# stjude-rust-labs/ngs

Measured on NVIDIA B200. Metric: ngs qc records/sec, higher is better.
Workload: dtype u8/u64

## Files before the change

ngs_b200/csrc/inflate2.cuh:

```cuda
#pragma once
#include <cstdint>
#include <cuda_runtime.h>

#include "inflate_lane.cuh"

namespace ngsq {

constexpr int kDecBatch = 32;
constexpr int kDecWarps = 18;
constexpr int kDecThreads = kDecWarps * 32;
constexpr size_t kDecSmem = (size_t)kDecThreads * kSlabBytes;

__global__ void __launch_bounds__(kDecThreads, 1)
inflate_decode_kernel(uint8_t* __restrict__ out, const BlockDesc* __restrict__ blocks, uint32_t n_blocks,
                      uint32_t* __restrict__ queue, uint32_t* __restrict__ status, uint32_t* __restrict__ bitmap) {
  extern __shared__ __align__(16) uint8_t smem_raw[];
  const uint32_t lane = threadIdx.x & 31;
  Lane L;
  L.slab = smem_raw + (size_t)threadIdx.x * kSlabBytes;
  L.state = LS_IDLE;
  __shared__ uint32_t s_base_lut[64];
  if (threadIdx.x < 64) s_base_lut[threadIdx.x] = base_lut_entry(threadIdx.x);
  __syncthreads();
  L.lut = s_base_lut;
  const uint32_t static_blocks = gridDim.x * (uint32_t)kDecWarps * 32u;
  bool first = true;
  for (;;) {
    uint32_t base = 0;
    if (first) {
      base = ((threadIdx.x >> 5) * gridDim.x + blockIdx.x) * 32u;
      first = false;
    } else {
      if (lane == 0) base = static_blocks + atomicAdd(queue, 32u);
      base = __shfl_sync(0xFFFFFFFFu, base, 0);
    }
    if (base >= n_blocks) break;
    const uint32_t b = base + lane;
    if (b < n_blocks) L.begin_block(blocks[b], out, bitmap + (size_t)b * kBitmapWords);
    else L.state = LS_IDLE;
    while (__any_sync(0xFFFFFFFFu, L.state != LS_IDLE)) {
      if (L.state == LS_HEADER) L.header();
      __syncwarp();
#pragma unroll 1
      for (int it = 0; it < kDecBatch; ++it) {
        if (L.state == LS_DECODE) L.step();
        L.settle();
        if (!__any_sync(0xFFFFFFFFu, L.state == LS_DECODE)) break;
      }
      if (L.state == LS_DECODE && L.overran()) L.end_block(kBlkBadStream);
    }
    if (b < n_blocks && L.err) status[b] = L.err;
  }
}

constexpr int kResThreads = 256;
constexpr int kResWarps = kResThreads / 32;
constexpr int kResList = 352;

__device__ __forceinline__ uint2 load8_unaligned(const uint8_t* s, uint32_t n) {
  const uint32_t* a = reinterpret_cast<const uint32_t*>(reinterpret_cast<uintptr_t>(s) & ~uintptr_t(3));
  const uint32_t mis = (uint32_t)(reinterpret_cast<uintptr_t>(s) & 3);
  const uint32_t sh = mis * 8;
  const uint32_t w0 = a[0], w1 = a[1];
  uint32_t w2 = 0;
  if (mis + n > 8) w2 = a[2];
  return make_uint2(__funnelshift_r(w0, w1, sh), __funnelshift_r(w1, w2, sh));
}

__device__ __forceinline__ void store_bytes(uint8_t* d, uint2 v, uint32_t n) {
  d[0] = (uint8_t)v.x;
  if (n > 1) d[1] = (uint8_t)(v.x >> 8);
  if (n > 2) d[2] = (uint8_t)(v.x >> 16);
  if (n > 3) d[3] = (uint8_t)(v.x >> 24);
  if (n > 4) d[4] = (uint8_t)v.y;
  if (n > 5) d[5] = (uint8_t)(v.y >> 8);
  if (n > 6) d[6] = (uint8_t)(v.y >> 16);
  if (n > 7) d[7] = (uint8_t)(v.y >> 24);
}

__device__ __forceinline__ void resolve_copy(uint8_t* dst, uint32_t mlen, uint32_t dist) {
  uint32_t D = dist;
  for (uint32_t done = 0; done < mlen;) {
    const uint32_t n = min(min(8u, D), mlen - done);
    store_bytes(dst + done, load8_unaligned(dst + done - D, n), n);
    done += n;
    if (D < 8) D <<= 1;
  }
}

__global__ void __launch_bounds__(kResThreads)
inflate_resolve_kernel(uint8_t* __restrict__ out, const BlockDesc* __restrict__ blocks, uint32_t n_blocks,
                       const uint32_t* __restrict__ bitmap, const uint32_t* __restrict__ status) {
  __shared__ uint16_t s_pos[kResWarps][kResList];
  __shared__ uint2 s_rank[kResWarps][32];
  const uint32_t lane = threadIdx.x & 31, wic = threadIdx.x >> 5;
  const uint32_t n_warps = gridDim.x * kResWarps;
  uint16_t* list = s_pos[wic];
  for (uint32_t b = blockIdx.x * kResWarps + wic; b < n_blocks; b += n_warps) {
    if (status[b]) continue;
    const BlockDesc d = blocks[b];
    uint8_t* ob = out + d.out_off;
    const uint32_t* bmp = bitmap + (size_t)b * kBitmapWords;
    const uint32_t n_sw = (d.isize + 1023) >> 10;
    for (uint32_t sw = 0; sw < n_sw; ++sw) {
      uint32_t word = bmp[sw * 32 + lane];
      const uint32_t cnt = __popc(word);
      uint32_t incl = cnt;
#pragma unroll
      for (int o = 1; o < 32; o <<= 1) {
        uint32_t t = __shfl_up_sync(0xFFFFFFFFu, incl, o);
        if ((int)lane >= o) incl += t;
      }
      const uint32_t total = __shfl_sync(0xFFFFFFFFu, incl, 31);
      if (!total) continue;
      uint32_t o = incl - cnt;
      s_rank[wic][lane] = make_uint2(word, o);
      const uint32_t pbase = (sw << 10) + (lane << 5);
      while (word) {
        const uint32_t bit = __ffs(word) - 1;
        word &= word - 1;
        list[o++] = (uint16_t)(pbase + bit);
      }
      __syncwarp();
      uint32_t pos_n = 0xFFFFu, tok_n = 0;
      if (lane < total) {
        pos_n = list[lane];
        const uint8_t* t = ob + pos_n;
        tok_n = (uint32_t)t[0] | ((uint32_t)t[1] << 8) | ((uint32_t)t[2] << 16);
      }
      for (uint32_t base = 0; base < total; base += 32) {
        const bool active = base + lane < total;
        const uint32_t pos = pos_n, tok = tok_n;
        const uint32_t jn = base + 32 + lane;
        if (jn < total) {
          pos_n = list[jn];
          const uint8_t* t = ob + pos_n;
          tok_n = (uint32_t)t[0] | ((uint32_t)t[1] << 8) | ((uint32_t)t[2] << 16);
        }
        const uint32_t mlen = (tok & 255u) + 3u, dist = (tok >> 8) + 1u;
        const uint32_t dend = active ? pos + mlen : 0x20000u;
        const uint32_t s_lo = pos - dist, s_hi = s_lo + min(mlen, dist);
        const uint32_t W = sw << 10;
        const uint32_t x_lo = min(max(s_lo, W) - W, 1023u), x_hi = min(max(s_hi, W) - W, 1023u);
        const uint2 e_lo = s_rank[wic][x_lo >> 5], e_hi = s_rank[wic][x_hi >> 5];
        const uint32_t r_lo = e_lo.y + __popc(e_lo.x & ((1u << (x_lo & 31)) - 1u));
        const uint32_t r_hi = e_hi.y + __popc(e_hi.x & ((1u << (x_hi & 31)) - 1u));
        const int pl = (int)r_lo - 1 - (int)base;
        const uint32_t prev_end = __shfl_sync(0xFFFFFFFFu, dend, pl & 31);
        const int lo = max((int)r_lo - (int)base - ((pl >= 0 && prev_end > s_lo) ? 1 : 0), 0), hi = (int)r_hi - (int)base;
        uint32_t dep = 0;
        if (active && hi > lo) dep = ((1u << hi) - 1u) & ~((1u << lo) - 1u) & ((1u << lane) - 1u);
        uint32_t done = __ballot_sync(0xFFFFFFFFu, !active);
        while (done != 0xFFFFFFFFu) {
          const bool ready = !((done >> lane) & 1u) && (dep & ~done) == 0;
          if (ready) resolve_copy(ob + pos, mlen, dist);
          __syncwarp();
          done |= __ballot_sync(0xFFFFFFFFu, ready);
        }
      }
      __syncwarp();
    }
  }
}

}
```

Measured before the change: 377.9 million.

## Interleave match copies chunk-wise across lanes and map one warp per block

The resolve kernel no longer runs a per-lane `resolve_copy` loop inside the warp's ready/ballot loop. Each ready lane now copies one chunk of at most 8 bytes per warp iteration, and a match is marked done only when its remaining length reaches zero. This removes the divergence where a whole warp waited on one long copy. The grid-stride loop is dropped in favour of one warp per BGZF block, launch bounds ask for 8 resident blocks per SM, and token loads and byte stores use word/mask forms. The one-warp-per-block mapping is correct only if the host launches enough blocks to cover every BGZF block; that launch code is not shown here.

```diff
diff --git a/ngs_b200/csrc/inflate2.cuh b/ngs_b200/csrc/inflate2.cuh
--- a/ngs_b200/csrc/inflate2.cuh
+++ b/ngs_b200/csrc/inflate2.cuh
@@ -68,98 +68,93 @@
 }
 
 __device__ __forceinline__ void store_bytes(uint8_t* d, uint2 v, uint32_t n) {
-  d[0] = (uint8_t)v.x;
-  if (n > 1) d[1] = (uint8_t)(v.x >> 8);
-  if (n > 2) d[2] = (uint8_t)(v.x >> 16);
-  if (n > 3) d[3] = (uint8_t)(v.x >> 24);
-  if (n > 4) d[4] = (uint8_t)v.y;
-  if (n > 5) d[5] = (uint8_t)(v.y >> 8);
-  if (n > 6) d[6] = (uint8_t)(v.y >> 16);
-  if (n > 7) d[7] = (uint8_t)(v.y >> 24);
+  const uint32_t m = (1u << n) - 1u;
+  if (m & 1u) d[0] = (uint8_t)v.x;
+  if (m & 2u) d[1] = (uint8_t)(v.x >> 8);
+  if (m & 4u) d[2] = (uint8_t)(v.x >> 16);
+  if (m & 8u) d[3] = (uint8_t)(v.x >> 24);
+  if (m & 16u) d[4] = (uint8_t)v.y;
+  if (m & 32u) d[5] = (uint8_t)(v.y >> 8);
+  if (m & 64u) d[6] = (uint8_t)(v.y >> 16);
+  if (m & 128u) d[7] = (uint8_t)(v.y >> 24);
 }
 
-__device__ __forceinline__ void resolve_copy(uint8_t* dst, uint32_t mlen, uint32_t dist) {
-  uint32_t D = dist;
-  for (uint32_t done = 0; done < mlen;) {
-    const uint32_t n = min(min(8u, D), mlen - done);
-    store_bytes(dst + done, load8_unaligned(dst + done - D, n), n);
-    done += n;
-    if (D < 8) D <<= 1;
-  }
-}
-
-__global__ void __launch_bounds__(kResThreads)
+__global__ void __launch_bounds__(kResThreads, 8)
 inflate_resolve_kernel(uint8_t* __restrict__ out, const BlockDesc* __restrict__ blocks, uint32_t n_blocks,
                        const uint32_t* __restrict__ bitmap, const uint32_t* __restrict__ status) {
   __shared__ uint16_t s_pos[kResWarps][kResList];
   __shared__ uint2 s_rank[kResWarps][32];
   const uint32_t lane = threadIdx.x & 31, wic = threadIdx.x >> 5;
-  const uint32_t n_warps = gridDim.x * kResWarps;
   uint16_t* list = s_pos[wic];
-  for (uint32_t b = blockIdx.x * kResWarps + wic; b < n_blocks; b += n_warps) {
-    if (status[b]) continue;
-    const BlockDesc d = blocks[b];
-    uint8_t* ob = out + d.out_off;
-    const uint32_t* bmp = bitmap + (size_t)b * kBitmapWords;
-    const uint32_t n_sw = (d.isize + 1023) >> 10;
-    for (uint32_t sw = 0; sw < n_sw; ++sw) {
-      uint32_t word = bmp[sw * 32 + lane];
-      const uint32_t cnt = __popc(word);
-      uint32_t incl = cnt;
+  const uint32_t b = blockIdx.x * kResWarps + wic;
+  if (b >= n_blocks || status[b]) return;
+  const BlockDesc d = blocks[b];
+  uint8_t* ob = out + d.out_off;
+  const uint32_t* bmp = bitmap + (size_t)b * kBitmapWords;
+  const uint32_t n_sw = (d.isize + 1023) >> 10;
+  for (uint32_t sw = 0; sw < n_sw; ++sw) {
+    uint32_t word = bmp[sw * 32 + lane];
+    const uint32_t cnt = __popc(word);
+    uint32_t incl = cnt;
 #pragma unroll
-      for (int o = 1; o < 32; o <<= 1) {
-        uint32_t t = __shfl_up_sync(0xFFFFFFFFu, incl, o);
-        if ((int)lane >= o) incl += t;
+    for (int o = 1; o < 32; o <<= 1) {
+      uint32_t t = __shfl_up_sync(0xFFFFFFFFu, incl, o);
+      if ((int)lane >= o) incl += t;
+    }
+    const uint32_t total = __shfl_sync(0xFFFFFFFFu, incl, 31);
+    if (!total) continue;
+    uint32_t o = incl - cnt;
+    s_rank[wic][lane] = make_uint2(word, o);
+    const uint32_t pbase = (sw << 10) + (lane << 5);
+    while (word) {
+      const uint32_t bit = __ffs(word) - 1;
+      word &= word - 1;
+      list[o++] = (uint16_t)(pbase + bit);
+    }
+    __syncwarp();
+    uint32_t pos_n = 0xFFFFu, tok_n = 0;
+    if (lane < total) {
+      pos_n = list[lane];
+      tok_n = load8_unaligned(ob + pos_n, 3).x & 0xFFFFFFu;
+    }
+    for (uint32_t base = 0; base < total; base += 32) {
+      const bool active = base + lane < total;
+      const uint32_t pos = pos_n, tok = tok_n;
+      const uint32_t jn = base + 32 + lane;
+      if (jn < total) {
+        pos_n = list[jn];
+        tok_n = load8_unaligned(ob + pos_n, 3).x & 0xFFFFFFu;
       }
-      const uint32_t total = __shfl_sync(0xFFFFFFFFu, incl, 31);
-      if (!total) continue;
-      uint32_t o = incl - cnt;
-      s_rank[wic][lane] = make_uint2(word, o);
-      const uint32_t pbase = (sw << 10) + (lane << 5);
-      while (word) {
-        const uint32_t bit = __ffs(word) - 1;
-        word &= word - 1;
-        list[o++] = (uint16_t)(pbase + bit);
+      const uint32_t mlen = (tok & 255u) + 3u, dist = (tok >> 8) + 1u;
+      const uint32_t dend = active ? pos + mlen : 0x20000u;
+      const uint32_t s_lo = pos - dist, s_hi = s_lo + min(mlen, dist);
+      const uint32_t W = sw << 10;
+      const uint32_t x_lo = min(max(s_lo, W) - W, 1023u), x_hi = min(max(s_hi, W) - W, 1023u);
+      const uint2 e_lo = s_rank[wic][x_lo >> 5], e_hi = s_rank[wic][x_hi >> 5];
+      const uint32_t r_lo = e_lo.y + __popc(e_lo.x & ((1u << (x_lo & 31)) - 1u));
+      const uint32_t r_hi = e_hi.y + __popc(e_hi.x & ((1u << (x_hi & 31)) - 1u));
+      const int pl = (int)r_lo - 1 - (int)base;
+      const uint32_t prev_end = __shfl_sync(0xFFFFFFFFu, dend, pl & 31);
+      const int lo = max((int)r_lo - (int)base - ((pl >= 0 && prev_end > s_lo) ? 1 : 0), 0), hi = (int)r_hi - (int)base;
+      uint32_t dep = 0;
+      if (active && hi > lo) dep = ((1u << hi) - 1u) & ~((1u << lo) - 1u) & ((1u << lane) - 1u);
+      uint8_t* dst = ob + pos;
+      uint32_t left = mlen, D = dist;
+      uint32_t done = __ballot_sync(0xFFFFFFFFu, !active);
+      while (done != 0xFFFFFFFFu) {
+        const bool ready = !((done >> lane) & 1u) && (dep & ~done) == 0;
+        if (ready) {
+          const uint32_t n = min(min(8u, D), left);
+          store_bytes(dst, load8_unaligned(dst - D, n), n);
+          dst += n;
+          left -= n;
+          if (D < 8) D <<= 1;
+        }
+        __syncwarp();
+        done |= __ballot_sync(0xFFFFFFFFu, ready && left == 0);
       }
-      __syncwarp();
-      uint32_t pos_n = 0xFFFFu, tok_n = 0;
-      if (lane < total) {
-        pos_n = list[lane];
-        const uint8_t* t = ob + pos_n;
-        tok_n = (uint32_t)t[0] | ((uint32_t)t[1] << 8) | ((uint32_t)t[2] << 16);
-      }
-      for (uint32_t base = 0; base < total; base += 32) {
-        const bool active = base + lane < total;
-        const uint32_t pos = pos_n, tok = tok_n;
-        const uint32_t jn = base + 32 + lane;
-        if (jn < total) {
-          pos_n = list[jn];
-          const uint8_t* t = ob + pos_n;
-          tok_n = (uint32_t)t[0] | ((uint32_t)t[1] << 8) | ((uint32_t)t[2] << 16);
-        }
-        const uint32_t mlen = (tok & 255u) + 3u, dist = (tok >> 8) + 1u;
-        const uint32_t dend = active ? pos + mlen : 0x20000u;
-        const uint32_t s_lo = pos - dist, s_hi = s_lo + min(mlen, dist);
-        const uint32_t W = sw << 10;
-        const uint32_t x_lo = min(max(s_lo, W) - W, 1023u), x_hi = min(max(s_hi, W) - W, 1023u);
-        const uint2 e_lo = s_rank[wic][x_lo >> 5], e_hi = s_rank[wic][x_hi >> 5];
-        const uint32_t r_lo = e_lo.y + __popc(e_lo.x & ((1u << (x_lo & 31)) - 1u));
-        const uint32_t r_hi = e_hi.y + __popc(e_hi.x & ((1u << (x_hi & 31)) - 1u));
-        const int pl = (int)r_lo - 1 - (int)base;
-        const uint32_t prev_end = __shfl_sync(0xFFFFFFFFu, dend, pl & 31);
-        const int lo = max((int)r_lo - (int)base - ((pl >= 0 && prev_end > s_lo) ? 1 : 0), 0), hi = (int)r_hi - (int)base;
-        uint32_t dep = 0;
-        if (active && hi > lo) dep = ((1u << hi) - 1u) & ~((1u << lo) - 1u) & ((1u << lane) - 1u);
-        uint32_t done = __ballot_sync(0xFFFFFFFFu, !active);
-        while (done != 0xFFFFFFFFu) {
-          const bool ready = !((done >> lane) & 1u) && (dep & ~done) == 0;
-          if (ready) resolve_copy(ob + pos, mlen, dist);
-          __syncwarp();
-          done |= __ballot_sync(0xFFFFFFFFu, ready);
-        }
-      }
-      __syncwarp();
     }
+    __syncwarp();
   }
 }
 
```

New measurement: 388.6 million (median of 6 runs). 2.8% higher.
